# ucla-brain/image-preprocessing-pipeline

Hardware: AMD Instinct MI355X
Metric: RL-deconv Gvoxels/sec (higher is better)
Workload: dtype f32; 1 GPU; c3: 2048x2048x512 fp32 volume, 31x31x61 PSF, deconFFT semantics, lambda=0, reg_interval=0; engine=fft, parallelism=single

## Files before the change

### image-preprocessing-pipeline_amd/capi.py

```python
from __future__ import annotations

import ctypes as C
import os

_HERE = os.path.dirname(os.path.abspath(__file__))
LIB_PATH = os.path.join(_HERE, "libmi_ipp_probes.so" if os.environ.get("MI_IPP_PROBES") == "1" else "libmi_ipp.so")

MI_OK = 0
IPC_HANDLE_BYTES = 64
BOUNDARY_ZERO, BOUNDARY_REPLICATE, BOUNDARY_CIRCULAR = 0, 1, 2
ENGINE_AUTO, ENGINE_DIRECT, ENGINE_FFT = 0, 1, 2
NORTH_SOUTH, WEST_EAST = 0, 1
SINBLEND, NOBLEND = 0, 1
HALVE_MEAN, HALVE_MAX = 0, 1
PS_U8, PS_U16, PS_F32 = 0, 1, 2
PS_PADDING = {"reflect": 0, "wrap": 1, "symmetric": 2, "edge": 3}
PS_DOWN = {"max": 0, "min": 1, "mean": 2}


MI_ERR_INVALID, MI_ERR_HIP, MI_ERR_FFT, MI_ERR_NOMEM, MI_ERR_UNSUPPORTED = -1, -2, -3, -4, -5


class MiError(RuntimeError):

# ... 66 lines not shown
                ("taps_x", C.c_int), ("tile_ny", C.c_int), ("tile_nx", C.c_int), ("lds_steps", C.c_int), ("scratch_bytes_per_slice", C.c_size_t)]


_vp, _i, _f, _sz = C.c_void_p, C.c_int, C.c_float, C.c_size_t
_ip = C.POINTER(C.c_int)

SIGNATURES = {
    "mi_last_error": (C.c_char_p, []),
    "mi_device_count": (_i, []),
    "mi_abi_version": (_i, []),
    "mi_stream_synchronize": (_i, [_i, _vp]),
    "mi_conv3d_replicate": (_i, [_i, _vp, _vp, _vp, _vp] + [_i] * 6),
    "mi_conv3d": (_i, [_i, _vp, _vp, _vp, _vp] + [_i] * 8),
    "mi_gauss3d_inplace": (_i, [_i, _vp, _vp, _vp, _i, _i, _i, C.POINTER(C.c_float), _ip]),
    "mi_edgetaper3d": (_i, [_i, _vp, _vp, _vp, _vp] + [_i] * 6),
    "mi_otf": (_i, [_i, _vp, _vp, _i, _i, _i, _vp, _i, _i, _i, _f]),
    "mi_u16_to_f32": (_i, [_i, _vp, _vp, _vp, _sz, _f]),
    "mi_subtract_dark": (_i, [_i, _vp, _vp, _vp, _sz, _f]),
    "mi_norm2": (_i, [_i, _vp, _vp, _sz, C.POINTER(C.c_double)]),
    "mi_release_cached_memory": (_sz, [_i]),
    "mi_cached_memory_bytes": (_sz, []),
    "mi_rl_fuses": (_i, [_vp]),
    "mi_rl_otf_is_real": (_i, [_vp]),
    "mi_rl_sharded_begin": (_i, [_vp, _vp, _vp]),
    "mi_rl_sharded_ratio": (_i, [_vp, _vp, _vp, _i, C.POINTER(C.c_int)]),
    "mi_rl_sharded_update": (_i, [_vp, _vp, _vp, _i, _i, C.POINTER(C.c_int)]),
    "mi_rl_spectrum_rows": (_i, [_vp, _vp, _i, _i, _vp, _i]),
    "mi_rl_spectrum_row_floats": (_sz, [_vp]),
    "mi_rl_sharded_stage": (_i, [_vp, _vp, _vp, _i, _i, _i, _i, C.POINTER(C.c_int)]),
    "mi_rl_spectrum_rows_z": (_i, [_vp, _vp, _i, _i, _i, _i, _vp, _i]),
    "mi_rl_z_granule": (_i, [_vp]),
    "mi_rl_set_overlap": (_i, [_vp, _i, _i]),
    "mi_rl_overlap_probe": (_i, [_vp, _vp, _vp, _ip, _i, _f, _i, C.POINTER(C.c_float)]),
    "mi_prctile": (_i, [_i, _vp, _vp, _sz, C.POINTER(C.c_double), _i, C.POINTER(C.c_float)]),
    "mi_rescale_block": (_i, [_i, _vp, _vp, _vp, _sz, _i, _f, _f, _f, _f]),
    "mi_pad_center": (_i, [_i, _vp, _vp, _i, _i, _i, _vp, _i, _i, _i]),
    "mi_crop_center": (_i, [_i, _vp, _vp, _i, _i, _i, _vp, _i, _i, _i]),
    "mi_rl_create": (_i, [_i, _vp, _i, _i, _i, _vp, _vp, _i, _i, _i, _i, _i, C.POINTER(_vp)]),
    "mi_rl_create_ex": (_i, [_i, _vp, _i, _i, _i, _vp, _vp, _i, _i, _i, _ip, _ip, _i, C.POINTER(_vp)]),
    "mi_rl_destroy": (_i, [_vp]),
    "mi_rl_engine": (_i, [_vp]),
    "mi_rl_separable": (_i, [_vp]),
    "mi_rl_pair_layout": (_i, [_vp]),
    "mi_rl_device_bytes": (_sz, [_vp]),
    "mi_rl_forward_ratio": (_i, [_vp, _vp, _vp, _vp]),
    "mi_rl_adjoint_update": (_i, [_vp, _vp, _vp, _vp, _f, _vp]),
# ... 132 lines not shown
```

### image-preprocessing-pipeline_amd/csrc/fft_native.h

```cpp
#pragma once
#include <vector>
#include <algorithm>
#include "conv3d_direct.h"

namespace mi {

struct NativeDims {
    int lhx2, r3x;
    int ly2, r3;
    int lz2, r3z;
    int hx, ny, nz;
    int ty, tc, tl;
    int z_in_hi, z_out_lo, z_out_hi, y_out_hi;
    int dbg;
    int paired;
    int zpad;
    int xrow;
    int xk0, xkn;
    int yz0;
    int xrot;
};

struct PadWindow {
    int on = 0;
// ... 2 lines not shown
    int rep[3] = {0, 0, 0};
    int w[3] = {0, 0, 0};
};

struct TileSelect {
    int mode = 0, lo0 = 0, n0 = 0, lo1 = 0, n1 = 0;
    int z0 = 0, nz = 0;
};

struct NoPlacementTrial {
    NoPlacementTrial();
    ~NoPlacementTrial();
    NoPlacementTrial(const NoPlacementTrial&) = delete;
    NoPlacementTrial& operator=(const NoPlacementTrial&) = delete;
    static bool active();
};

struct NativeFft {
    NativeDims dims{};
    DevBuf S, G, G_adj, tw;
    float2* t_spec = nullptr;
    DevBuf Gr, Gr_adj, ph;
    bool real_otf = false;
    bool have_adj = false;
    const float2* tw_x = nullptr;
    const float2* tw_y = nullptr;
    const float2* tw_z = nullptr;
    size_t n_cplx = 0;
    size_t spec_bytes = 0;
    int n_cu = 256;
    ~NativeFft();

    static bool supported(const int F[3]);
    static int good_size(int n, int axis);
    int init(hipStream_t s, const int F[3], bool explicit_adjoint);
    int build_otf(hipStream_t s, const float* placed, bool adjoint_slot, float scale);
    int spectrum(hipStream_t s, const float* vol, float4* dst, float scale);
    size_t otf_items() const { return G.bytes / sizeof(float4); }
    float4* otf() { return G.as<float4>(); }
    int try_real_otf(hipStream_t s, const int delta[3]);
    float* scratch() { return reinterpret_cast<float*>(t_spec); }
    void set_window(const int n[3], const int o[3], const int rep[3], const int k[3]);
    bool can_fuse() const;
    int conv(hipStream_t s, const float* in, bool conj_otf, float* out, int epi_kind, const ConvEpilogue& epi);
    int iterate(hipStream_t s, float* bl, int n_iters);
    size_t spectrum_bytes() const { return spec_bytes; }
    size_t spectrum_row_floats() const { return (size_t)2 * dims.nz * dims.hx; }
    size_t device_bytes() const {
        return S.bytes + place.T2.bytes + place.S_alt.bytes + G.bytes + G_adj.bytes + Gr.bytes + Gr_adj.bytes + ph.bytes + tw.bytes;
    }

    int x_forward(hipStream_t s, const float* in);
    int middle(hipStream_t s, bool conj_otf);
    int y_pass(hipStream_t s, bool inverse, bool paired, const float2* src = nullptr, float2* dst = nullptr, int xk0 = 0, int xkn = -1);
    int z_conv(hipStream_t s, bool conj_otf, const float2* src = nullptr, float2* dst = nullptr, int xk0 = 0, int xkn = -1);
    int x_inverse(hipStream_t s, float* out, int epi_kind, const ConvEpilogue& epi, bool fuse_forward, const TileSelect* part = nullptr);
    bool z_pipelined() const;
    int spectrum_rows(hipStream_t s, int y0, int rows, float2* buf, int dir, int z0 = 0, int nzc = 0);
    int y_forward_planes(hipStream_t s, int z0, int nzc);
    int y_z_granule() const { return dims.paired ? std::max(1, dims.tc / 2) : 1; }

    PadWindow pw{};
    bool pipe_ok() const;
    bool splits() const;
    TileSelect edge_tiles(int mode, int a0, int a1, int b0, int b1) const;
    bool pad_pipe(bool aligned) const;
    int pipe_tiles(bool padded, const TileSelect* part, TileSelect* sel, int* ntiles) const;
    int x_pipelined(hipStream_t s, int mode, const float2* T, float* out, const ConvEpilogue& epi, int ek, const TileSelect& sel, int ntiles);
    int overlap_free_cus = 0;
    bool overlap_dynamic = true;
    bool x_dynamic = true;
    DevBuf ctr;
// ... 22 lines not shown
```

### image-preprocessing-pipeline_amd/csrc/fft_native_dev.h

```cpp
#pragma once
#include <cmath>
#include <cstdlib>
#include <type_traits>
#include <vector>

#include "fft_native.h"

namespace mi {
namespace {

#ifndef MI_FFT_UNROLL
#define MI_FFT_UNROLL 4
#endif
constexpr int kThreadsXZ = 1024;
constexpr int kWavesXZ = 4;
constexpr int kThreadsY = 512;
#ifndef MI_YCUT
#define MI_YCUT 1
#endif
constexpr int kYCut = MI_YCUT;

__host__ __device__ constexpr int swz_g(int t) { return ((t & 1) ? 15 : 0) ^ ((t & 2) ? 13 : 0) ^ ((t & 4) ? 25 : 0) ^ ((t & 8) ? 16 : 0); }
__host__ __device__ constexpr int swz_c(int i) { return i ^ swz_g((i >> 4) & 15); }
__host__ __device__ constexpr unsigned long long swz_table_hi() {
// ... 47 lines not shown
}
__device__ __forceinline__ float2 cmulc(float2 a, float2 b) {
    const v2f A = V2(a), B = V2(b);
    const v2f axx = __builtin_shufflevector(A, A, 0, 0), ayy = __builtin_shufflevector(A, A, 1, 1);
    const v2f bc = {B.x, -B.y}, bsw = {B.y, B.x};
    return F2(__builtin_elementwise_fma(ayy, bsw, axx * bc));
}
__device__ __forceinline__ float2 cadd(float2 a, float2 b) { return F2(V2(a) + V2(b)); }
__device__ __forceinline__ float2 csub(float2 a, float2 b) { return F2(V2(a) - V2(b)); }
__device__ __forceinline__ float2 cconj(float2 a) { return make_float2(a.x, -a.y); }
__device__ __forceinline__ unsigned brev_n(unsigned v, int bits) { return bits == 0 ? 0u : (__brev(v) >> (32 - bits)); }

__device__ __forceinline__ int pos2freq(int p, int l2, int r3) {
    const int k1 = p >> l2, pp = p & ((1 << l2) - 1);
    return k1 + r3 * (int)brev_n((unsigned)pp, l2);
}
__device__ __forceinline__ int freq2pos(int k, int l2, int r3) {
    const int k2 = k / r3, k1 = k - k2 * r3;
    return (k1 << l2) + (int)brev_n((unsigned)k2, l2);
}
__device__ __forceinline__ int mirror_pos(int p, int n, int l2, int r3) {
    const int k = pos2freq(p, l2, r3);
    return freq2pos(k == 0 ? 0 : n - k, l2, r3);
}
__host__ __device__ constexpr bool x_rotated(int lhx2, int r3) { return r3 == 1 && (lhx2 == 10 || lhx2 == 11); }
__device__ __forceinline__ int x_work2pos(int w, const NativeDims& d) {
    const int r = 3 * d.xrot, s = d.xrot * (d.lhx2 - 3);
    return ((w & ((1 << r) - 1)) << s) | (w >> r);
}
__device__ __forceinline__ int x_pos2work(int p, const NativeDims& d) {
    const int r = 3 * d.xrot, s = d.xrot * (d.lhx2 - 3);
    return ((p & ((1 << s) - 1)) << r) | (p >> s);
}
__device__ __forceinline__ int x_freq2pos(int k, const NativeDims& d) { return x_work2pos(freq2pos(k, d.lhx2, d.r3x), d); }
__device__ __forceinline__ int y_pos2freq(int p, const NativeDims& d) { return pos2freq(p, d.ly2, d.r3); }
__device__ __forceinline__ int y_mirror_pos(int p, const NativeDims& d) { return mirror_pos(p, d.ny, d.ly2, d.r3); }

__device__ __forceinline__ int pad_src(const PadWindow& p, int a, int g) {
    if (p.rep[a]) return g < p.w[a] ? min(max(g - p.o[a], 0), p.n[a] - 1) : -1;
    const int s = g - p.o[a];
    return (s >= 0 && s < p.n[a]) ? s : -1;
}
__device__ __forceinline__ int pad_dst(const PadWindow& p, int a, int g) {
    const int s = g - p.o[a];
    return (s >= 0 && s < p.n[a]) ? s : -1;
}
// ... 401 lines not shown
```

### image-preprocessing-pipeline_amd/csrc/fft_native_place.hip

```cpp
#include <mutex>

#include "fft_native.h"

namespace mi {

namespace {
thread_local int tl_no_placement_trial = 0;
}
NoPlacementTrial::NoPlacementTrial() { ++tl_no_placement_trial; }
NoPlacementTrial::~NoPlacementTrial() { --tl_no_placement_trial; }
bool NoPlacementTrial::active() { return tl_no_placement_trial != 0; }

int NativeFft::place_by_trial(hipStream_t s, size_t gap) {
    const int Hx = dims.hx;
    const size_t n_buf = spec_bytes / sizeof(float2);
    int tries = 6;
    if (const char* e = std::getenv("MI_FFT_PLACE_CANDIDATES")) tries = std::max(1, std::min(8, atoi(e)));
    static std::mutex trial_mu[16];
    int dev_id = 0;
    MI_HIP(hipGetDevice(&dev_id));
    std::lock_guard<std::mutex> trial_lock(trial_mu[dev_id & 15]);
    (void)mi_release_cached_memory(dev_id);
    size_t free_b = 0, total_b = 0;
    MI_HIP(hipMemGetInfo(&free_b, &total_b));
// ... 155 lines not shown
            case 1: return y_pass(s, false, dims.paired != 0);
            case 2: return z_conv(s, false);
            default: return y_pass(s, true, dims.paired != 0);
        }
    });
}

int NativeFft::time_between(hipStream_t s, int which, const float2* src, float2* dst, float* bl, int reps, float* avg_ms) {
    void* const s_own = S.p;
    float2* const t_own = t_spec;
    ConvEpilogue ep;
    ep.a = bl;
    return timed_launches(s, reps, "time_between", avg_ms, [&] {
        int rc;
        if (which == 0) {
            rc = y_pass(s, false, dims.paired != 0, src, dst);
        } else if (which == 2) {
            S.p = dst;
            rc = x_forward(s, bl);
            S.p = s_own;
        } else if (which == 3) {
            rc = z_conv(s, false, src, dst);
        } else if (which == 4) {
            void* const g_own = Gr.p;
            if (!g_own) return fail(MI_ERR_UNSUPPORTED, "time_between: no real OTF");
            Gr.p = const_cast<float2*>(src);
            rc = z_conv(s, false);
            Gr.p = g_own;
        } else {
            t_spec = const_cast<float2*>(src);
            S.p = dst;
            rc = x_inverse(s, bl, EPI_UPDATE, ep, true);
            S.p = s_own;
            t_spec = t_own;
        }
        return rc;
    });
}

}
```

### image-preprocessing-pipeline_amd/csrc/fft_native_yz.hip

```cpp
#include "fft_native_dev.h"

namespace mi {
namespace {

template <int LY2, int R3, bool INVERSE>
__global__ __launch_bounds__(kThreadsY, 4) void k_y_pass(const float2* __restrict__ src, float2* __restrict__ dst, NativeDims d,
                                                      const float2* __restrict__ tw) {
    extern __shared__ __attribute__((aligned(16))) float2 tile[];
    constexpr int M = R3 << LY2, NW = kThreadsY / 64;
    constexpr int pitch = row_pitch(M), quads = M / 2;
    constexpr int TCC = y_tile_cols(M);
    const int TC = d.tc, Hx = d.hx, L = d.nz;
    const size_t c0 = (size_t)blockIdx.x * TC + (INVERSE ? (size_t)0 : (size_t)d.yz0 * Hx);
    if (!INVERSE) {
        if ((int)(c0 / Hx) >= d.z_in_hi) return;
    } else if (L % TC == 0) {
        const int z_first = (int)(c0 % L);
        if (z_first >= d.z_out_hi || z_first + TC <= d.z_out_lo) return;
    }
    const size_t src_pitch = INVERSE ? (size_t)M : (size_t)d.xrow, dst_pitch = INVERSE ? (size_t)d.xrow : (size_t)M;
    const float4* base = reinterpret_cast<const float4*>(src + c0 * src_pitch);
    const bool priv = (TC % NW) == 0;
    using TW = TwLds<LY2, R3, kYCut>;
    float2* twl = tile + TC * pitch;
// ... 552 lines not shown
        const bool self_plane = (w.px == w.pxB);
        const FView fv = f_view();
        float4* dA = reinterpret_cast<float4*>(T + (size_t)w.px * L * M + w.py0) + fv.off;
        float4* dB = reinterpret_cast<float4*>(T + (size_t)w.pxB * L * M + w.pyB0) + fv.off;
#pragma unroll
        for (int k = 0; k < NPA; ++k) {
            const int zk = fv.z0 + k * P;
            if ((NA % kThreadsXZ == 0 || (int)threadIdx.x + k * kThreadsXZ < NA) && zk >= d.z_out_lo && zk < d.z_out_hi) {
                const int cA = fv.row + (fv.slot ^ swz_c(k * P));
                int cB0 = cA + TL * pitch, cB1 = cB0 + pitch;
                if constexpr (WP) b_cells(ptab, fv.jp, fv.pz ^ swz_c(k * P), cB0, cB1);
                const float2 a0 = tile[cA], a1 = tile[cA + pitch];
                dA[(size_t)(k * P) * rowq] = make_float4(a0.x, a0.y, a1.x, a1.y);
                if (!self_plane) {
                    const float2 b0 = tile[cB0], b1 = tile[cB1];
                    dB[(size_t)(k * P) * rowq] = make_float4(b0.x, b0.y, b1.x, b1.y);
                }
            }
        }
        lds_barrier();
    }
}

template <int LZ2, int R3, bool REALG, int NT, int TL, bool PHL = true, bool TOPON = true>
__global__ __launch_bounds__(NT, (NT == 512 && (R3 << LZ2) > 576) ? 2 : kWavesXZ) void k_z_pair_pipe(const float2* __restrict__ S, float2* __restrict__ T, const float4* __restrict__ G,
                                                              NativeDims d, const float2* __restrict__ tw, int conj_otf, int ntiles, RealOtf ro,
                                                              int* __restrict__ tile_ctr) {
    extern __shared__ __attribute__((aligned(16))) float2 tile[];
    __shared__ int s_next_tile;
    constexpr int L = R3 << LZ2, NW = NT / 64, hp = TL, pitch = row_pitch(L);
    constexpr bool WP = TL == NW;
    static_assert((WP || (NW == 2 * TL && L % 128 == 0)) && L % 64 == 0 && (TL * L) % NT == 0, "one or two waves per line pair");
    constexpr int NPA = TL * L / NT;
    constexpr int P = NT / TL;
    constexpr int NPG = TL * L / NT;
    constexpr int TOPS = seg_below(LZ2, LZ2), TOPR = LZ2 - TOPS;
    constexpr bool TOPREG = TOPON && R3 == 1 && (1 << TOPS) == P && (1 << TOPR) == NPA;
    const int Hx = d.hx, M = d.ny, ytiles = M / TL;
    const size_t ZR = (size_t)(M + d.zpad);
    struct FView { int row, slot, z0; size_t off; };
    auto f_view = [&]() {
        const int tid = launder(threadIdx.x);
        const int z0 = tid / TL, jq = tid - z0 * TL;
        return FView{(2 * jq) * pitch, phys(z0) ^ rmask(2 * jq, hp), z0, (size_t)z0 * ZR + jq};
    };
    float4 pre[NPA];
    auto load_S = [&](int t) {
        const int pl = t / ytiles, ty = t - pl * ytiles, plane = d.xk0 + pl;
        const FView fv = f_view();
        const float4* sp = reinterpret_cast<const float4*>(S) + (size_t)plane * L * ZR + (size_t)ty * TL + fv.off;
#pragma unroll
        for (int k = 0; k < NPA; ++k) pre[k] = (fv.z0 + k * P < d.z_in_hi) ? sp[(size_t)(k * P) * ZR] : make_float4(0.0f, 0.0f, 0.0f, 0.0f);
    };
    using TW = TwLds<LZ2, R3>;
    float2* twl = tile + 2 * TL * pitch;
// ... 30 lines not shown
                    tile[c] = v[k];
                    tile[c + pitch] = u[k];
                }
            } else {
#pragma unroll
            for (int k = 0; k < NPA; ++k) {
                const int c = fv.row + (fv.slot ^ swz_c(k * P));
                tile[c] = make_float2(pre[k].x, pre[k].y);
                tile[c + pitch] = make_float2(pre[k].z, pre[k].w);
            }
            }
        }
        const size_t g0 = ((size_t)plane * M + py0) * L;
        float4 gv[REALG ? 1 : NPG];
        float2 gr[REALG ? NPG : 1];
        float2 ph_xy = make_float2(1.0f, 0.0f);
        auto load_G = [&]() {
            const int tid = launder(threadIdx.x);
            const int wv = __builtin_amdgcn_readfirstlane(tid >> 6);
            const int line = WP ? wv : wv % TL, p0 = WP ? 0 : (wv / TL) * (L / 2);
            if constexpr (REALG) {
                ph_xy = cmul(ro.ph_x[plane], ro.ph_y[y_pos2freq(py0 + line, d)]);
            }
            const size_t gl = g0 + (size_t)line * L + p0 + (tid & 63);
#pragma unroll
            for (int k = 0; k < NPG; ++k) {
                if constexpr (REALG) gr[k] = ro.g[gl + 64 * k];
                else gv[k] = G[gl + 64 * k];
            }
        };
        constexpr bool LATE_G = !REALG && R3 == 1 && !TOPREG && LZ2 - seg_below(LZ2, LZ2) == 4;
        if (R3 != 9 && !LATE_G) load_G();
        lds_barrier();
        if constexpr (R3 > 1) {
            radix3_stage<R3, false, NT>(tile, 2 * TL, pitch, hp, true, 1 << LZ2, twl + TW::r3);
            wave_lds_fence();
        }
        if (R3 == 9) load_G();
        if constexpr (LATE_G) {
            lds_fft<LZ2, false, NT, R3, 0, 4>(tile, 2 * TL * R3, pitch, hp, true, twl);
            load_G();
            lds_fft<LZ2, false, NT, R3, 4, LZ2>(tile, 2 * TL * R3, pitch, hp, true, twl);
        } else {
            lds_fft<LZ2, false, NT, R3, TOPREG ? TOPR : 0>(tile, 2 * TL * R3, pitch, hp, true, twl);
        }
        if constexpr (!WP) lds_barrier();
        float sw, cw;
        sincospif(-2.0f * (float)plane / (float)(2 * Hx), &sw, &cw);
        const float2 wx = make_float2(cw, sw);
        {
            const int tid = launder(threadIdx.x);
            const int wv = __builtin_amdgcn_readfirstlane(tid >> 6);
            const int lane = tid & 63;
            const int line = WP ? wv : wv % TL, p0 = WP ? 0 : (wv / TL) * (L / 2);
            const int pA = phys(lane) ^ rmask(line, hp), pB1 = phys(lane ^ 63) ^ rmask(TL + line, hp);
            const int pB0 = phys(mirror_pos(lane, L, LZ2, R3)) ^ rmask(TL + line, hp);
#pragma unroll
            for (int k = 0; k < NPG; ++k) {
                const int hb = 64 * k + p0;
                const int cA = line * pitch + (pA ^ swz_c(hb));
                int cB;
                if constexpr (R3 == 1) {
                    const int flo = (int)brev_n((unsigned)hb, LZ2);
                    const int mhi = flo ? (int)brev_n((unsigned)((1 << (LZ2 - 6)) - flo), LZ2) : 0;
                    cB = (TL + line) * pitch + (flo ? (pB1 ^ swz_c(mhi)) : pB0);
                } else {
                    cB = (TL + line) * pitch + (phys(mirror_pos(lane + hb, L, LZ2, R3)) ^ rmask(TL + line, hp));
                }
                const float2 a = tile[cA];
                const float2 bc = cconj(tile[cB]);
                const float2 E = make_float2(0.5f * (a.x + bc.x), 0.5f * (a.y + bc.y));
                const float2 dlt = csub(a, bc);
                const float2 O = make_float2(0.5f * dlt.y, -0.5f * dlt.x);
                const float2 wO = cmul(wx, O);
                const float2 Xa = cadd(E, wO), Xb = csub(E, wO);
                float2 Ya, Yb;
                if constexpr (REALG) {
                    float2 Pq = cmul(ph_xy, PHL ? phl[lane + hb] : ro.ph_z[pos2freq(lane + hb, LZ2, R3)]);
                    if (conj_otf) Pq.y = -Pq.y;
                    const float2 XaP = cmul(Xa, Pq), XbP = cmul(Xb, Pq);
                    Ya = make_float2(XaP.x * gr[k].x, XaP.y * gr[k].x);
                    Yb = make_float2(XbP.x * gr[k].y, XbP.y * gr[k].y);
                } else {
                    float2 Ga = make_float2(gv[k].x, gv[k].y), Gb = make_float2(gv[k].z, gv[k].w);
                    if (conj_otf) { Ga.y = -Ga.y; Gb.y = -Gb.y; }
                    Ya = cmul(Xa, Ga);
                    Yb = cmul(Xb, Gb);
                }
                const float2 E2 = make_float2(0.5f * (Ya.x + Yb.x), 0.5f * (Ya.y + Yb.y));
                const float2 dY = csub(Ya, Yb);
                const float2 O2 = cmulc(make_float2(0.5f * dY.x, 0.5f * dY.y), wx);
                tile[cA] = make_float2(E2.x - O2.y, E2.y + O2.x);
                tile[cB] = make_float2(E2.x + O2.y, O2.x - E2.y);
            }
        }
        if (R3 != 9 && tn < ntiles) load_S(tn);
        if constexpr (WP) wave_lds_fence();
        else lds_barrier();
        lds_fft<LZ2, true, NT, R3, 0, TOPREG ? TOPS : LZ2>(tile, 2 * TL * R3, pitch, hp, true, twl);
        if constexpr (R3 > 1) {
            radix3_stage<R3, true, NT>(tile, 2 * TL, pitch, hp, true, 1 << LZ2, twl + TW::r3);
            wave_lds_fence();
        }
        if (R3 == 9 && tn < ntiles) load_S(tn);
        lds_barrier();
// ... 34 lines not shown
        tn = dyn ? __builtin_amdgcn_readfirstlane(s_next_tile) : tn + (int)gridDim.x;
    }
}

__global__ __launch_bounds__(256) void k_g_to_real(const float4* __restrict__ G, float2* __restrict__ Gr, NativeDims d, RealOtf ro,
                                                    size_t total, unsigned* __restrict__ stats) {
    const int M = d.ny, L = d.nz;
    float max_im = 0.0f, max_re = 0.0f;
    for (size_t i = blockIdx.x * (size_t)blockDim.x + threadIdx.x; i < total; i += (size_t)gridDim.x * blockDim.x) {
        const int pz = (int)(i % L);
        const size_t r = i / L;
        const int py = (int)(r % M), xk = (int)(r / M);
        const float2 P = cmul(cmul(ro.ph_x[xk], ro.ph_y[y_pos2freq(py, d)]), ro.ph_z[pos2freq(pz, d.lz2, d.r3z)]);
        const float4 g = G[i];
        const float2 a = cmulc(make_float2(g.x, g.y), P), b = cmulc(make_float2(g.z, g.w), P);
        Gr[i] = make_float2(a.x, b.x);
        max_im = fmaxf(max_im, fmaxf(fabsf(a.y), fabsf(b.y)));
        max_re = fmaxf(max_re, fmaxf(fabsf(a.x), fabsf(b.x)));
    }
    atomicMax(&stats[0], __float_as_uint(max_im));
    atomicMax(&stats[1], __float_as_uint(max_re));
}

RealOtf real_otf_args(const NativeFft& f, bool adj_slot) {
    RealOtf ro{};
    ro.g = adj_slot ? f.Gr_adj.as<float2>() : f.Gr.as<float2>();
    ro.ph_x = f.ph.as<float2>();
    ro.ph_y = ro.ph_x + (f.dims.hx / 2 + 1);
    ro.ph_z = ro.ph_y + f.dims.ny;
    return ro;
}

#define MI_ZQ_CASES(M) M(6, 1, 512, true) M(7, 1, 512, true) M(8, 1, 512, true) M(9, 1, 512, true) M(10, 1, 512, true) \
    M(6, 3, 512, true) M(7, 3, 512, true) M(8, 3, 1024, true) M(6, 9, 512, false) M(7, 9, 1024, true)
#define MI_ZQ_CALL(LG, R, NTH, PH) case LG * 16 + R: return f(Int<LG>{}, Int<R>{}, Int<NTH>{}, std::bool_constant<PH>{});
template <class F>
int z_pair_case(const NativeDims& d, F&& f) {
    switch (d.lz2 * 16 + d.r3z) { MI_ZQ_CASES(MI_ZQ_CALL) default: return fail(MI_ERR_UNSUPPORTED, "native FFT: paired z length %d", d.nz); }
}
#undef MI_ZQ_CALL

}

int NativeFft::y_pass(hipStream_t s, bool inverse, bool paired, const float2* src_o, float2* dst_o, int xk0, int xkn) {
    const int Hx = dims.hx, L = dims.nz;
    if (xkn < 0) xkn = Hx / 2 + 1;
    MI_REQUIRE(paired || (xk0 == 0 && xkn == Hx / 2 + 1), "native FFT: only the paired y pass runs on a chunk of planes");
    const unsigned ycols = paired ? (unsigned)((size_t)xkn * (L / (dims.tc / 2))) : (unsigned)((size_t)L * Hx / dims.tc);
    NativeDims d = dims;
// ... 20 lines not shown
    const int Hx = dims.hx, M = dims.ny, L = dims.nz;
    if (xkn < 0) xkn = Hx / 2 + 1;
    MI_REQUIRE(dims.paired || (xk0 == 0 && xkn == Hx / 2 + 1), "native FFT: only the paired z pass runs on a chunk of planes");
    const unsigned ztiles = (unsigned)((size_t)(Hx / 2 + 1) * (M / dims.tl));
    const size_t zl = lds_bytes(2 * dims.tl, L);
    NativeDims d = dims;
    d.xk0 = xk0;
    d.xkn = xkn;
    const float2* Tp = src_o ? src_o : t_spec;
    float2* Sp = dst_o ? dst_o : S.as<float2>();
    const bool adj_slot = conj_otf && have_adj;
    const float4* Gp = adj_slot ? G_adj.as<float4>() : G.as<float4>();
    const float2* twz = tw_z;
    const int cj = (conj_otf && !have_adj) ? 1 : 0;
    const RealOtf ro = real_otf ? real_otf_args(*this, adj_slot) : RealOtf{};
    if (dims.paired) {
        const int ntiles = xkn * (M / kPairLines);
        const bool phl = !(dims.lz2 == 6 && dims.r3z == 9);
        const size_t lds = lds_bytes(2 * kPairLines, L) + (real_otf && phl ? sizeof(float2) * (size_t)L : 0);
        const int per_cu = std::max(1, std::min(2, (int)(kLdsOneWg / lds)));
        const unsigned grid = (unsigned)std::min(ntiles, per_cu * n_cu);
        int* ctr_p = nullptr;
        {
            static const char* env_dyn = std::getenv("MI_Z_DYN");
            if (env_dyn ? atoi(env_dyn) != 0 : z_dynamic) {
                if (!ctr.p) MI_TRY(ctr.alloc(256));
                ctr_p = ctr.as<int>() + 16 + 4 * (ctr_slot & 7);
                MI_HIP(hipMemsetAsync(ctr_p, 0, sizeof(int), s));
            }
        }
        return z_pair_case(dims, [&](auto lg, auto r, auto nth, auto ph_lds) {
            constexpr int LG = lg(), R = r(), NTH = nth();
            constexpr bool PH = ph_lds();
            return real_otf ? launch_lds(k_z_pair_pipe<LG, R, true, NTH, kPairLines, PH>, grid, NTH, lds, s, "k_z_pair_pipe<real OTF>", Tp, Sp, Gp,
                                         d, twz, cj, ntiles, ro, ctr_p)
                            : launch_lds(k_z_pair_pipe<LG, R, false, NTH, kPairLines, PH>, grid, NTH, lds, s, "k_z_pair_pipe", Tp, Sp, Gp, d,
                                         twz, cj, ntiles, ro, ctr_p);
        });
    }
    if (z_pipelined()) {
        const int ntiles = (int)ztiles;
        const unsigned grid = (unsigned)std::min(ntiles, n_cu);
        return z_case(dims, [&](auto lg, auto r) {
            constexpr int LG = lg(), R = r();
            if constexpr (z_pipe_even(R << LG)) {
                if (real_otf)
                    return launch_lds(k_z_conv_pipe<LG, R, true>, grid, kThreadsXZ, zl, s, "k_z_conv_pipe<real OTF>", Tp, Sp, Gp, d, twz, cj, ntiles, ro);
            }
            return launch_lds(k_z_conv_pipe<LG, R, false>, grid, kThreadsXZ, zl, s, "k_z_conv_pipe", Tp, Sp, Gp, d, twz, cj, ntiles, ro);
        });
    }
    MI_REQUIRE(!real_otf, "native FFT: the real OTF form needs the pipelined z pass");
    return z_case(dims, [&](auto lg, auto r) {
        return launch_lds(k_z_conv<lg(), r(), false>, ztiles, kThreadsXZ, zl, s, "k_z_conv", Tp, Sp, Gp, d, twz, cj, (float4*)nullptr, 0.0f);
    });
}
// ... 24 lines not shown
    MI_HIP(hipMemcpyAsync(ph.p, h.data(), sizeof(float2) * h.size(), hipMemcpyHostToDevice, s));
    const RealOtf ro = real_otf_args(*this, false);
    const size_t total = (size_t)nx * M * L;
    DevBuf st;
    MI_TRY(st.alloc(4 * sizeof(unsigned)));
    MI_HIP(hipMemsetAsync(st.p, 0, 4 * sizeof(unsigned), s));
    size_t blocks = (total + 255) / 256;
    if (blocks > 256 * 16) blocks = 256 * 16;
    for (int slot = 0; slot < (have_adj ? 2 : 1); ++slot) {
        DevBuf& dst = slot ? Gr_adj : Gr;
        MI_TRY(dst.alloc(sizeof(float2) * total));
        hipLaunchKernelGGL(k_g_to_real, dim3((unsigned)blocks), dim3(256), 0, s, (slot ? G_adj : G).as<float4>(), dst.as<float2>(), dims, ro,
                           total, st.as<unsigned>() + 2 * slot);
        MI_TRY(launch_check("k_g_to_real"));
    }
    float hs[4] = {0, 0, 0, 0};
    MI_HIP(hipMemcpyAsync(hs, st.p, sizeof(hs), hipMemcpyDeviceToHost, s));
    MI_HIP(hipStreamSynchronize(s));
    bool ok = hs[0] <= 4e-6f * hs[1] && (!have_adj || hs[2] <= 4e-6f * hs[3]);
    if (ok) {
        real_otf = true;
        G.release();
        G_adj.release();
    } else {
        Gr.release();
        Gr_adj.release();
        ph.release();
    }
    return MI_OK;
}

int NativeFft::build_otf(hipStream_t s, const float* placed, bool adjoint_slot, float scale) {
    MI_REQUIRE(!adjoint_slot || have_adj, "native FFT: no adjoint OTF slot");
    return spectrum(s, placed, adjoint_slot ? G_adj.as<float4>() : G.as<float4>(), scale);
}

int NativeFft::spectrum(hipStream_t s, const float* vol, float4* Gp, float scale) {
    MI_REQUIRE(!pw.on, "native FFT: spectra are taken on the unpadded grid (before the pad window is set)");
    MI_TRY(x_forward(s, vol));
    MI_TRY(y_pass(s, false, false));
    const unsigned ztiles = (unsigned)((size_t)(dims.hx / 2 + 1) * (dims.ny / dims.tl));
    return z_case(dims, [&](auto lg, auto r) {
        return launch_lds(k_z_conv<lg(), r(), true>, ztiles, kThreadsXZ, lds_bytes(2 * dims.tl, dims.nz), s, "k_z_conv<build>", (const float2*)t_spec,
                          S.as<float2>(), (const float4*)nullptr, dims, tw_z, 0, Gp, scale);
    });
}

}
```

### image-preprocessing-pipeline_amd/csrc/rl.hip

```cpp
#include <chrono>
#include <cmath>
#include <cstring>
#include <new>
#include <utility>
#include <vector>

#include "fftconv.h"

using namespace mi;

struct mi_rl_ctx {
    int dev = 0;
    int n[3] = {0, 0, 0};
    int k[3] = {0, 0, 0};
    int bnd[3] = {MI_BOUNDARY_ZERO, MI_BOUNDARY_ZERO, MI_BOUNDARY_ZERO};
    int engine = MI_ENGINE_DIRECT;
    DevBuf kf_fwd, kf_adj;
    int kxp = 0;
    int off_fwd[3] = {0, 0, 0}, off_adj[3] = {0, 0, 0};
    bool separable = false;
    DevBuf sep_fwd[3], sep_adj[3];
    int sep_kxp[3] = {0, 0, 0};
    DevBuf sep_t0, sep_t1;
    SepTaps sep_tf[3], sep_ta[3];
// ... 268 lines not shown
extern "C" int mi_fft_good_size(int n, int axis) {
    if (axis < 0 || axis > 2 || n < 1) return 0;
    return NativeFft::good_size(n, axis);
}

static int sharded_native(mi_rl_ctx* ctx, NativeFft** out) {
    MI_REQUIRE(ctx, "mi_rl_sharded: null context");
    MI_TRY(use_device(ctx->dev));
    if (!(ctx->engine == MI_ENGINE_FFT && ctx->fft->native && ctx->fft->native->can_fuse()))
        return fail(MI_ERR_UNSUPPORTED, "mi_rl_sharded: only the native FFT pipeline fuses consecutive convolutions");
    *out = ctx->fft->native;
    return ctx->fft->native->release_spare();
}

extern "C" int mi_rl_fuses(mi_rl_ctx* ctx) {
    if (!(ctx && ctx->engine == MI_ENGINE_FFT && ctx->fft->native && ctx->fft->native->can_fuse())) return 0;
    return ctx->fft->native->splits() ? 2 : 1;
}

extern "C" int mi_rl_otf_is_real(mi_rl_ctx* ctx) {
    return ctx && ctx->engine == MI_ENGINE_FFT && ctx->fft->native && ctx->fft->native->real_otf ? 1 : 0;
}

extern "C" int mi_rl_sharded_begin(mi_rl_ctx* ctx, void* stream, const float* bl) {
    NativeFft* nf = nullptr;
    MI_TRY(sharded_native(ctx, &nf));
    MI_REQUIRE(bl, "mi_rl_sharded_begin: null pointer");
    return nf->x_forward(as_stream(stream), bl);
}

static int sharded_step(mi_rl_ctx* ctx, void* stream, float* bl, bool update, int more, int part, const int* edges) {
    NativeFft* nf = nullptr;
    MI_TRY(sharded_native(ctx, &nf));
    MI_REQUIRE(bl, "mi_rl_sharded: null pointer");
    MI_REQUIRE(part >= 0 && part <= 2, "mi_rl_sharded: part must be 0, 1 or 2");
    TileSelect sel{};
    if (part != 0) {
        MI_REQUIRE(nf->splits(), "mi_rl_sharded: this context cannot split the x pass (mi_rl_fuses() != 2)");
        MI_REQUIRE(edges && edges[0] >= 0 && edges[0] < edges[1] && edges[1] <= edges[2] && edges[2] < edges[3] && edges[3] <= ctx->n[1],
                   "mi_rl_sharded: edge row ranges must be ordered and inside the volume");
        sel = nf->edge_tiles(part, edges[0], edges[1], edges[2], edges[3]);
    }
    ConvEpilogue e;
    e.a = bl;
    if (part != 2) MI_TRY(nf->middle(as_stream(stream), update));
    return update ? nf->x_inverse(as_stream(stream), bl, EPI_UPDATE, e, more != 0, &sel)
// ... 627 lines not shown
```

### image-preprocessing-pipeline_amd/decon.py

```python
from __future__ import annotations

import ctypes as C
from types import SimpleNamespace

import numpy as np
import torch

from . import capi
from .capi import (BOUNDARY_CIRCULAR, BOUNDARY_REPLICATE, BOUNDARY_ZERO, ENGINE_AUTO, ENGINE_DIRECT, ENGINE_FFT,
                   RlOptions, check, lib)

__all__ = ["decon", "conv3d_gpu", "convn_same", "gauss3d_gpu", "edgetaper_3d", "otf_gpu", "im2single", "RLContext",
           "make_psf_struct", "norm2", "prctile", "rescale_block", "pad_block_to_fft_shape", "unpad_block", "next_fast_len", "engine_select"]


def _device(device_id=None) -> torch.device:
    capi.require_gpu()
    if device_id is None:
        return torch.device("cuda", torch.cuda.current_device())
    if isinstance(device_id, torch.device):
        return device_id
    if int(device_id) <= 0:
        raise ValueError("device_id 0 selects the reference's MATLAB CPU path, which this build does not contain")
    return torch.device("cuda", int(device_id) - 1)
# ... 244 lines not shown
            self._chk(ratio)
        check(lib().mi_rl_iterate(self._h, _stream(bl), bl.data_ptr(), ratio.data_ptr() if ratio is not None else None,
                                  int(n_iters)))

    @property
    def fuses(self) -> int:
        return int(lib().mi_rl_fuses(self._h))

    @property
    def separable(self) -> bool:
        return bool(lib().mi_rl_separable(self._h))

    @property
    def separable_single_pass(self) -> bool:
        return int(lib().mi_rl_separable(self._h)) == 2

    @property
    def pair_layout(self) -> bool:
        return bool(lib().mi_rl_pair_layout(self._h))

    @property
    def otf_is_real(self) -> bool:
        return bool(lib().mi_rl_otf_is_real(self._h))

    @property
    def spectrum_row_floats(self) -> int:
        return int(lib().mi_rl_spectrum_row_floats(self._h))

    def sharded_begin(self, bl):
        self._chk(bl)
        check(lib().mi_rl_sharded_begin(self._h, _stream(bl), bl.data_ptr()))

    @staticmethod
    def _edges(edge_rows):
        return (C.c_int * 4)(*[int(v) for v in edge_rows]) if edge_rows is not None else None

    def sharded_ratio(self, bl, part=0, edge_rows=None):
        self._chk(bl)
        check(lib().mi_rl_sharded_ratio(self._h, _stream(bl), bl.data_ptr(), int(part), self._edges(edge_rows)))

    def sharded_update(self, bl, more=True, part=0, edge_rows=None):
        self._chk(bl)
        check(lib().mi_rl_sharded_update(self._h, _stream(bl), bl.data_ptr(), int(bool(more)), int(part), self._edges(edge_rows)))

    def set_overlap(self, free_cus=0, dynamic_tiles=False):
        check(lib().mi_rl_set_overlap(self._h, int(free_cus), int(bool(dynamic_tiles))))
# ... 145 lines not shown
```

### include/mi_lsdeconv.h

```cpp
#ifndef MI_LSDECONV_H
#define MI_LSDECONV_H

#include "mi_common.h"

#ifdef __cplusplus
extern "C" {
#endif

typedef enum {
    MI_BOUNDARY_ZERO = 0,
    MI_BOUNDARY_REPLICATE = 1,
    MI_BOUNDARY_CIRCULAR = 2
} mi_boundary;

typedef enum {
    MI_ENGINE_AUTO = 0,
    MI_ENGINE_DIRECT = 1,
    MI_ENGINE_FFT = 2
} mi_engine;


int mi_conv3d_replicate(int dev, void* stream, const float* img, const float* ker, float* out,
                        int nx, int ny, int nz, int kx, int ky, int kz);

// ... 25 lines not shown

int mi_pad_center(int dev, void* stream, const float* src, int nx, int ny, int nz, float* dst, int fx, int fy, int fz);
int mi_crop_center(int dev, void* stream, const float* src, int fx, int fy, int fz, float* dst, int nx, int ny, int nz);


typedef struct mi_rl_ctx mi_rl_ctx;

int mi_rl_create(int dev, void* stream, int nx, int ny, int nz, const float* psf, const float* psf_inv,
                 int kx, int ky, int kz, int boundary, int engine, mi_rl_ctx** ctx);
int mi_rl_create_ex(int dev, void* stream, int nx, int ny, int nz, const float* psf, const float* psf_inv,
                    int kx, int ky, int kz, const int* boundary_xyz, const int* shift_xyz, int engine,
                    mi_rl_ctx** ctx);
int mi_rl_separable(const mi_rl_ctx* ctx);
int mi_rl_pair_layout(const mi_rl_ctx* ctx);
int mi_rl_destroy(mi_rl_ctx* ctx);
int mi_rl_engine(const mi_rl_ctx* ctx);
size_t mi_rl_device_bytes(const mi_rl_ctx* ctx);

int mi_rl_forward_ratio(mi_rl_ctx* ctx, void* stream, const float* bl, float* ratio);
int mi_rl_adjoint_update(mi_rl_ctx* ctx, void* stream, const float* ratio, float* bl, float lambda, const float* reg);
int mi_rl_iterate(mi_rl_ctx* ctx, void* stream, float* bl, float* ratio, int n_iters);
int mi_rl_fuses(mi_rl_ctx* ctx);
int mi_rl_otf_is_real(mi_rl_ctx* ctx);
int mi_rl_sharded_begin(mi_rl_ctx* ctx, void* stream, const float* bl);
int mi_rl_sharded_ratio(mi_rl_ctx* ctx, void* stream, const float* bl, int part, const int* edge_rows);
int mi_rl_sharded_update(mi_rl_ctx* ctx, void* stream, float* bl, int more, int part, const int* edge_rows);
int mi_rl_spectrum_rows(mi_rl_ctx* ctx, void* stream, int y0, int rows, float* buf, int dir);
size_t mi_rl_spectrum_row_floats(mi_rl_ctx* ctx);
int mi_rl_sharded_stage(mi_rl_ctx* ctx, void* stream, float* bl, int update, int stage, int z0, int z1, const int* edge_rows);
int mi_rl_spectrum_rows_z(mi_rl_ctx* ctx, void* stream, int y0, int rows, int z0, int z1, float* buf, int dir);
int mi_rl_z_granule(mi_rl_ctx* ctx);
int mi_rl_set_overlap(mi_rl_ctx* ctx, int free_cus, int dynamic_tiles);
int mi_rl_overlap_probe(mi_rl_ctx* ctx, void* stream, float* bl, const int* edge_rows, int busy_wgs, float busy_us, int reps,
                        float* out_ms);
int mi_rl_time_pass(mi_rl_ctx* ctx, void* stream, int which, const float* bl, int reps, float* avg_ms);
size_t mi_rl_fft_spectrum_bytes(mi_rl_ctx* ctx);
int mi_rl_time_between(mi_rl_ctx* ctx, void* stream, int which, const void* src, void* dst, float* bl, int reps, float* avg_ms);
int mi_rl_fft_placement(mi_rl_ctx* ctx, float* cost_ms, int cap, int* n, int* kept);
int mi_rl_reg_term(int dev, void* stream, const float* bl, float* reg, int nx, int ny, int nz);


typedef struct {
    int niter;
    float lambda;
    float stop_criterion;
    int regularize_interval;
// ... 56 lines not shown
```

Baseline: 71.25 Gvoxel*iter/s.

## Fold the real OTF along z using mirror symmetry to halve its reads

When the real-form OTF is symmetric in z (checked at build time against a tolerance), only about half of each z line is stored in a compacted pitch. The paired z pass loads the kept half and rebuilds the mirrored half with a cross-lane ds_bpermute. This cuts OTF memory traffic in the z convolution pass. In exchange it adds a fold kernel and a host sync at setup, and the mirrored half is an approximation that is only accepted within the tolerance.

```diff
diff --git a/image-preprocessing-pipeline_amd/capi.py b/image-preprocessing-pipeline_amd/capi.py
--- a/image-preprocessing-pipeline_amd/capi.py
+++ b/image-preprocessing-pipeline_amd/capi.py
@@ -112,6 +112,8 @@
     "mi_cached_memory_bytes": (_sz, []),
     "mi_rl_fuses": (_i, [_vp]),
     "mi_rl_otf_is_real": (_i, [_vp]),
+    "mi_rl_otf_folded": (_i, [_vp]),
+    "mi_fft_otf_fold_slot": (_i, [_i, _i]),
     "mi_rl_sharded_begin": (_i, [_vp, _vp, _vp]),
     "mi_rl_sharded_ratio": (_i, [_vp, _vp, _vp, _i, C.POINTER(C.c_int)]),
     "mi_rl_sharded_update": (_i, [_vp, _vp, _vp, _i, _i, C.POINTER(C.c_int)]),
diff --git a/image-preprocessing-pipeline_amd/csrc/fft_native.h b/image-preprocessing-pipeline_amd/csrc/fft_native.h
--- a/image-preprocessing-pipeline_amd/csrc/fft_native.h
+++ b/image-preprocessing-pipeline_amd/csrc/fft_native.h
@@ -48,6 +48,8 @@
     float2* t_spec = nullptr;
     DevBuf Gr, Gr_adj, ph;
     bool real_otf = false;
+    DevBuf Gf, Gf_adj;
+    bool otf_fold = false;
     bool have_adj = false;
     const float2* tw_x = nullptr;
     const float2* tw_y = nullptr;
@@ -65,6 +67,7 @@
     size_t otf_items() const { return G.bytes / sizeof(float4); }
     float4* otf() { return G.as<float4>(); }
     int try_real_otf(hipStream_t s, const int delta[3]);
+    int try_otf_fold(hipStream_t s, const float max_re[2]);
     float* scratch() { return reinterpret_cast<float*>(t_spec); }
     void set_window(const int n[3], const int o[3], const int rep[3], const int k[3]);
     bool can_fuse() const;
@@ -73,7 +76,7 @@
     size_t spectrum_bytes() const { return spec_bytes; }
     size_t spectrum_row_floats() const { return (size_t)2 * dims.nz * dims.hx; }
     size_t device_bytes() const {
-        return S.bytes + place.T2.bytes + place.S_alt.bytes + G.bytes + G_adj.bytes + Gr.bytes + Gr_adj.bytes + ph.bytes + tw.bytes;
+        return S.bytes + place.T2.bytes + place.S_alt.bytes + G.bytes + G_adj.bytes + Gr.bytes + Gr_adj.bytes + Gf.bytes + Gf_adj.bytes + ph.bytes + tw.bytes;
     }
 
     int x_forward(hipStream_t s, const float* in);
diff --git a/image-preprocessing-pipeline_amd/csrc/fft_native_dev.h b/image-preprocessing-pipeline_amd/csrc/fft_native_dev.h
--- a/image-preprocessing-pipeline_amd/csrc/fft_native_dev.h
+++ b/image-preprocessing-pipeline_amd/csrc/fft_native_dev.h
@@ -93,6 +93,30 @@
 __device__ __forceinline__ int mirror_pos(int p, int n, int l2, int r3) {
     const int k = pos2freq(p, l2, r3);
     return freq2pos(k == 0 ? 0 : n - k, l2, r3);
+}
+__host__ __device__ constexpr int otf_fold_entries(int n) { return n <= 64 ? n : 64 + (n - 64) / 2; }
+__host__ __device__ constexpr int otf_fold_pitch(int n) { return (otf_fold_entries(n) + 15) & ~15; }
+__host__ __device__ constexpr int otf_fold_slot(int l2, int p) {
+    (void)l2;
+    if (p < 64) return p;
+    int m = 6;
+    while ((2 << m) <= p) ++m;
+    const int half = 1 << (m - 1);
+    int q = p - (1 << m);
+    if (q >= half) q = 2 * half - 1 - q;
+    return 32 + half + q;
+}
+__host__ __device__ constexpr int otf_fold_mirror(int p) {
+    if (p < 2) return p;
+    int m = 1;
+    while ((2 << m) <= p) ++m;
+    return p ^ ((1 << m) - 1);
+}
+__host__ __device__ constexpr bool otf_fold_kept(int p) {
+    if (p < 64) return true;
+    int m = 6;
+    while ((2 << m) <= p) ++m;
+    return p - (1 << m) < (1 << (m - 1));
 }
 __host__ __device__ constexpr bool x_rotated(int lhx2, int r3) { return r3 == 1 && (lhx2 == 10 || lhx2 == 11); }
 __device__ __forceinline__ int x_work2pos(int w, const NativeDims& d) {
diff --git a/image-preprocessing-pipeline_amd/csrc/fft_native_place.hip b/image-preprocessing-pipeline_amd/csrc/fft_native_place.hip
--- a/image-preprocessing-pipeline_amd/csrc/fft_native_place.hip
+++ b/image-preprocessing-pipeline_amd/csrc/fft_native_place.hip
@@ -201,11 +201,12 @@
         } else if (which == 3) {
             rc = z_conv(s, false, src, dst);
         } else if (which == 4) {
-            void* const g_own = Gr.p;
+            DevBuf& g = otf_fold ? Gf : Gr;
+            void* const g_own = g.p;
             if (!g_own) return fail(MI_ERR_UNSUPPORTED, "time_between: no real OTF");
-            Gr.p = const_cast<float2*>(src);
+            g.p = const_cast<float2*>(src);
             rc = z_conv(s, false);
-            Gr.p = g_own;
+            g.p = g_own;
         } else {
             t_spec = const_cast<float2*>(src);
             S.p = dst;
diff --git a/image-preprocessing-pipeline_amd/csrc/fft_native_yz.hip b/image-preprocessing-pipeline_amd/csrc/fft_native_yz.hip
--- a/image-preprocessing-pipeline_amd/csrc/fft_native_yz.hip
+++ b/image-preprocessing-pipeline_amd/csrc/fft_native_yz.hip
@@ -598,7 +598,7 @@
     }
 }
 
-template <int LZ2, int R3, bool REALG, int NT, int TL, bool PHL = true, bool TOPON = true>
+template <int LZ2, int R3, bool REALG, int NT, int TL, bool PHL = true, bool TOPON = true, bool FOLD = false>
 __global__ __launch_bounds__(NT, (NT == 512 && (R3 << LZ2) > 576) ? 2 : kWavesXZ) void k_z_pair_pipe(const float2* __restrict__ S, float2* __restrict__ T, const float4* __restrict__ G,
                                                               NativeDims d, const float2* __restrict__ tw, int conj_otf, int ntiles, RealOtf ro,
                                                               int* __restrict__ tile_ctr) {
@@ -607,6 +607,7 @@
     constexpr int L = R3 << LZ2, NW = NT / 64, hp = TL, pitch = row_pitch(L);
     constexpr bool WP = TL == NW;
     static_assert((WP || (NW == 2 * TL && L % 128 == 0)) && L % 64 == 0 && (TL * L) % NT == 0, "one or two waves per line pair");
+    static_assert(!FOLD || (REALG && R3 == 1 && WP && L >= 128), "the folded OTF: real form, 2^a lines owned by one wave");
     constexpr int NPA = TL * L / NT;
     constexpr int P = NT / TL;
     constexpr int NPG = TL * L / NT;
@@ -683,11 +684,22 @@
             if constexpr (REALG) {
                 ph_xy = cmul(ro.ph_x[plane], ro.ph_y[y_pos2freq(py0 + line, d)]);
             }
+            if constexpr (FOLD) {
+                const int lane = tid & 63;
+                const float2* gp = ro.g + ((size_t)plane * M + py0 + line) * otf_fold_pitch(L);
+                gr[0] = gp[lane];
+                gr[1] = gp[64 + min(lane, 63 - lane)];
+#pragma unroll
+                for (int k = 2; k < NPG; ++k) {
+                    if (otf_fold_kept(64 * k)) gr[k] = gp[otf_fold_slot(LZ2, 64 * k) + lane];
+                }
+            } else {
             const size_t gl = g0 + (size_t)line * L + p0 + (tid & 63);
 #pragma unroll
             for (int k = 0; k < NPG; ++k) {
                 if constexpr (REALG) gr[k] = ro.g[gl + 64 * k];
                 else gv[k] = G[gl + 64 * k];
+            }
             }
         };
         constexpr bool LATE_G = !REALG && R3 == 1 && !TOPREG && LZ2 - seg_below(LZ2, LZ2) == 4;
@@ -721,10 +733,18 @@
                 const int hb = 64 * k + p0;
                 const int cA = line * pitch + (pA ^ swz_c(hb));
                 int cB;
+                float2 gk = gr[REALG ? k : 0];
                 if constexpr (R3 == 1) {
                     const int flo = (int)brev_n((unsigned)hb, LZ2);
                     const int mhi = flo ? (int)brev_n((unsigned)((1 << (LZ2 - 6)) - flo), LZ2) : 0;
                     cB = (TL + line) * pitch + (flo ? (pB1 ^ swz_c(mhi)) : pB0);
+                    if constexpr (FOLD) {
+                        if (k >= 2 && !otf_fold_kept(hb)) {
+                            const float2 gm = gr[otf_fold_mirror(hb) >> 6];
+                            gk.x = __int_as_float(__builtin_amdgcn_ds_bpermute((63 - lane) << 2, __float_as_int(gm.x)));
+                            gk.y = __int_as_float(__builtin_amdgcn_ds_bpermute((63 - lane) << 2, __float_as_int(gm.y)));
+                        }
+                    }
                 } else {
                     cB = (TL + line) * pitch + (phys(mirror_pos(lane + hb, L, LZ2, R3)) ^ rmask(TL + line, hp));
                 }
@@ -740,8 +760,8 @@
                     float2 Pq = cmul(ph_xy, PHL ? phl[lane + hb] : ro.ph_z[pos2freq(lane + hb, LZ2, R3)]);
                     if (conj_otf) Pq.y = -Pq.y;
                     const float2 XaP = cmul(Xa, Pq), XbP = cmul(Xb, Pq);
-                    Ya = make_float2(XaP.x * gr[k].x, XaP.y * gr[k].x);
-                    Yb = make_float2(XbP.x * gr[k].y, XbP.y * gr[k].y);
+                    Ya = make_float2(XaP.x * gk.x, XaP.y * gk.x);
+                    Yb = make_float2(XbP.x * gk.y, XbP.y * gk.y);
                 } else {
                     float2 Ga = make_float2(gv[k].x, gv[k].y), Gb = make_float2(gv[k].z, gv[k].w);
                     if (conj_otf) { Ga.y = -Ga.y; Gb.y = -Gb.y; }
@@ -822,9 +842,25 @@
     atomicMax(&stats[1], __float_as_uint(max_re));
 }
 
+__global__ __launch_bounds__(256) void k_g_fold(const float2* __restrict__ Gr, float2* __restrict__ Gf, NativeDims d, size_t total,
+                                                 unsigned* __restrict__ stats) {
+    const int L = d.nz, pitchf = otf_fold_pitch(L);
+    float max_d = 0.0f;
+    for (size_t i = blockIdx.x * (size_t)blockDim.x + threadIdx.x; i < total; i += (size_t)gridDim.x * blockDim.x) {
+        const int pz = (int)(i % L);
+        if (!otf_fold_kept(pz)) continue;
+        const size_t line = i / L;
+        const float2 a = Gr[i], b = Gr[line * L + mirror_pos(pz, L, d.lz2, 1)];
+        Gf[line * pitchf + otf_fold_slot(d.lz2, pz)] = a;
+        max_d = fmaxf(max_d, fmaxf(fabsf(a.x - b.x), fabsf(a.y - b.y)));
+    }
+    atomicMax(&stats[0], __float_as_uint(max_d));
+}
+
 RealOtf real_otf_args(const NativeFft& f, bool adj_slot) {
     RealOtf ro{};
-    ro.g = adj_slot ? f.Gr_adj.as<float2>() : f.Gr.as<float2>();
+    if (f.otf_fold) ro.g = adj_slot ? f.Gf_adj.as<float2>() : f.Gf.as<float2>();
+    else ro.g = adj_slot ? f.Gr_adj.as<float2>() : f.Gr.as<float2>();
     ro.ph_x = f.ph.as<float2>();
     ro.ph_y = ro.ph_x + (f.dims.hx / 2 + 1);
     ro.ph_z = ro.ph_y + f.dims.ny;
@@ -891,7 +927,7 @@
         const unsigned grid = (unsigned)std::min(ntiles, per_cu * n_cu);
         int* ctr_p = nullptr;
         {
-            static const char* env_dyn = std::getenv("MI_Z_DYN");
+            const char* env_dyn = std::getenv("MI_Z_DYN");
             if (env_dyn ? atoi(env_dyn) != 0 : z_dynamic) {
                 if (!ctr.p) MI_TRY(ctr.alloc(256));
                 ctr_p = ctr.as<int>() + 16 + 4 * (ctr_slot & 7);
@@ -901,6 +937,12 @@
         return z_pair_case(dims, [&](auto lg, auto r, auto nth, auto ph_lds) {
             constexpr int LG = lg(), R = r(), NTH = nth();
             constexpr bool PH = ph_lds();
+            if constexpr (R == 1 && LG >= 7) {
+                if (otf_fold)
+                    return launch_lds(k_z_pair_pipe<LG, R, true, NTH, kPairLines, PH, true, true>, grid, NTH, lds, s, "k_z_pair_pipe<folded OTF>",
+                                      Tp, Sp, Gp, d, twz, cj, ntiles, ro, ctr_p);
+            }
+            MI_REQUIRE(!otf_fold, "native FFT: the folded OTF needs the paired z pass of 2^a lines");
             return real_otf ? launch_lds(k_z_pair_pipe<LG, R, true, NTH, kPairLines, PH>, grid, NTH, lds, s, "k_z_pair_pipe<real OTF>", Tp, Sp, Gp,
                                          d, twz, cj, ntiles, ro, ctr_p)
                             : launch_lds(k_z_pair_pipe<LG, R, false, NTH, kPairLines, PH>, grid, NTH, lds, s, "k_z_pair_pipe", Tp, Sp, Gp, d,
@@ -971,12 +1013,50 @@
         real_otf = true;
         G.release();
         G_adj.release();
+        const float max_re[2] = {hs[1], hs[3]};
+        MI_TRY(try_otf_fold(s, max_re));
     } else {
         Gr.release();
         Gr_adj.release();
         ph.release();
     }
     return MI_OK;
+}
+
+int NativeFft::try_otf_fold(hipStream_t s, const float max_re[2]) {
+    const int M = dims.ny, L = dims.nz, nx = dims.hx / 2 + 1;
+    if (std::getenv("MI_FFT_NO_OTF_FOLD") != nullptr || !dims.paired || dims.r3z != 1 || L < 128) return MI_OK;
+    const size_t total = (size_t)nx * M * L, folded = (size_t)nx * M * otf_fold_pitch(L);
+    const int slots = have_adj ? 2 : 1;
+    DevBuf st;
+    MI_TRY(st.alloc(2 * sizeof(unsigned)));
+    MI_HIP(hipMemsetAsync(st.p, 0, 2 * sizeof(unsigned), s));
+    size_t blocks = (total + 255) / 256;
+    if (blocks > 256 * 16) blocks = 256 * 16;
+    for (int slot = 0; slot < slots; ++slot) {
+        DevBuf& dst = slot ? Gf_adj : Gf;
+        MI_TRY(dst.alloc(sizeof(float2) * folded));
+        hipLaunchKernelGGL(k_g_fold, dim3((unsigned)blocks), dim3(256), 0, s, (slot ? Gr_adj : Gr).as<float2>(), dst.as<float2>(), dims, total,
+                           st.as<unsigned>() + slot);
+        MI_TRY(launch_check("k_g_fold"));
+    }
+    float hd[2] = {0, 0};
+    MI_HIP(hipMemcpyAsync(hd, st.p, sizeof(hd), hipMemcpyDeviceToHost, s));
+    MI_HIP(hipStreamSynchronize(s));
+    if (hd[0] <= 4e-6f * max_re[0] && (!have_adj || hd[1] <= 4e-6f * max_re[1])) {
+        otf_fold = true;
+        Gr.release();
+        Gr_adj.release();
+    } else {
+        Gf.release();
+        Gf_adj.release();
+    }
+    return MI_OK;
+}
+
+extern "C" int mi_fft_otf_fold_slot(int lz2, int p) {
+    if (lz2 < 6 || lz2 > 10 || p < 0 || p >= (1 << lz2)) return -1;
+    return otf_fold_slot(lz2, p);
 }
 
 int NativeFft::build_otf(hipStream_t s, const float* placed, bool adjoint_slot, float scale) {
diff --git a/image-preprocessing-pipeline_amd/csrc/rl.hip b/image-preprocessing-pipeline_amd/csrc/rl.hip
--- a/image-preprocessing-pipeline_amd/csrc/rl.hip
+++ b/image-preprocessing-pipeline_amd/csrc/rl.hip
@@ -314,6 +314,10 @@
     return ctx && ctx->engine == MI_ENGINE_FFT && ctx->fft->native && ctx->fft->native->real_otf ? 1 : 0;
 }
 
+extern "C" int mi_rl_otf_folded(mi_rl_ctx* ctx) {
+    return ctx && ctx->engine == MI_ENGINE_FFT && ctx->fft->native && ctx->fft->native->otf_fold ? 1 : 0;
+}
+
 extern "C" int mi_rl_sharded_begin(mi_rl_ctx* ctx, void* stream, const float* bl) {
     NativeFft* nf = nullptr;
     MI_TRY(sharded_native(ctx, &nf));
diff --git a/image-preprocessing-pipeline_amd/decon.py b/image-preprocessing-pipeline_amd/decon.py
--- a/image-preprocessing-pipeline_amd/decon.py
+++ b/image-preprocessing-pipeline_amd/decon.py
@@ -290,6 +290,10 @@
     @property
     def otf_is_real(self) -> bool:
         return bool(lib().mi_rl_otf_is_real(self._h))
+
+    @property
+    def otf_folded(self) -> bool:
+        return bool(lib().mi_rl_otf_folded(self._h))
 
     @property
     def spectrum_row_floats(self) -> int:
diff --git a/include/mi_lsdeconv.h b/include/mi_lsdeconv.h
--- a/include/mi_lsdeconv.h
+++ b/include/mi_lsdeconv.h
@@ -71,6 +71,8 @@
 int mi_rl_iterate(mi_rl_ctx* ctx, void* stream, float* bl, float* ratio, int n_iters);
 int mi_rl_fuses(mi_rl_ctx* ctx);
 int mi_rl_otf_is_real(mi_rl_ctx* ctx);
+int mi_rl_otf_folded(mi_rl_ctx* ctx);
+int mi_fft_otf_fold_slot(int lz2, int p);
 int mi_rl_sharded_begin(mi_rl_ctx* ctx, void* stream, const float* bl);
 int mi_rl_sharded_ratio(mi_rl_ctx* ctx, void* stream, const float* bl, int part, const int* edge_rows);
 int mi_rl_sharded_update(mi_rl_ctx* ctx, void* stream, float* bl, int more, int part, const int* edge_rows);
```

Result: no change. 71.05 Gvoxel*iter/s (-0.3%).
